# NinV/Background-Debiased-Video-CIL

Hardware: AMD Instinct MI355X
Metric: clips/sec fwd+bwd TSM-R50 8x224^2 bs32/GPU (higher is better)
Workload: dtype f32; 1 GPU; TSM-ResNet50 fwd+bwd+SGD step, synthetic 32x8x3x224x224 clips per GPU, 101 classes, SimpleLinear+CrossEntropyLoss, dropout 0.5, random-init weights; fp32 tensors, accumulators and results; conv products: fp32 via 3xbf16 split, 6 MFMA products, fp32 accumulate (dropped terms <= 2^-24 relative); conv_arith=bf16x3, clips_per_gpu=32, global_batch=32, parallelism=dp1

## Files before the change

background-debiased-video-cil_amd/_lib.py:

```python
from __future__ import annotations

import ctypes
import os
from ctypes import POINTER, Structure, c_char, c_char_p, c_float, c_int, c_int32, c_int64, c_size_t, c_uint16, c_uint64, c_void_p

_HERE = os.path.dirname(os.path.abspath(__file__))
_OVERRIDE = os.environ.get('BDVCIL_LIB_PATH')
LIB_PATH = _OVERRIDE or os.path.join(_HERE, 'csrc', 'libbdvcil_hip.so')
ABI_VERSION = 33

_lib = None


class ConvGeom(Structure):
    _fields_ = [(n, c_int32) for n in
                ('N', 'H', 'W', 'Cin', 'Ho', 'Wo', 'Cout', 'R', 'S', 'stride', 'pad', 'T', 'fold', 'pad_w', 'Rt', 'st_t', 'act_dtype')]

    def key(self):
        return tuple(getattr(self, n) for n, _ in self._fields_)


class ConvPlan(Structure):
    _fields_ = [(n, c_int32) for n in ('family', 'reads_planes', 'stat_rows', 'splits', 'pre_ok')] + [('kernel', c_char * 128)]

# ... 19 lines not shown
        return (self.width, self.height, self.ncomp, tuple(self.h), tuple(self.v))


SIGNATURES = {
    'bdv_last_error': (c_char_p, []),
    'bdv_abi_version': (c_int, []),
    'bdv_source_hash': (c_char_p, []),
    'bdv_conv_workspace_bytes': (c_size_t, [POINTER(ConvGeom), c_int]),
    'bdv_conv_plan_query': (c_int, [POINTER(ConvGeom), c_int, c_int, c_int, POINTER(ConvPlan)]),
    'bdv_conv_fprop': (c_int, [P, P, P, POINTER(ConvGeom), P, POINTER(ConvAffine), P, c_size_t, P]),
    'bdv_conv_dgrad': (c_int, [P, P, P, P, P, POINTER(ConvGeom), POINTER(BnStatFuse), P, c_size_t, P]),
    'bdv_conv_weight_planes_bytes': (c_size_t, [POINTER(ConvGeom)]),
    'bdv_conv_split_weights': (c_int, [P, POINTER(ConvGeom), P, P, P]),
    'bdv_conv_debug_force_tile': (c_int, [c_int]),
    'bdv_conv_debug_row_run': (c_int, [c_int]),
    'bdv_conv_fprop_pl': (c_int, [P, P, P, P, POINTER(ConvGeom), P, POINTER(ConvAffine), P, c_size_t, c_int, P, P, P]),
    'bdv_conv_dgrad_pl': (c_int, [P, P, P, P, P, P, POINTER(ConvGeom), POINTER(BnStatFuse), P, c_size_t, c_int, P]),
    'bdv_conv_wgrad': (c_int, [P, P, P, c_float, POINTER(ConvGeom), P, c_size_t, P]),
    'bdv_conv_wgrad_partial': (c_int, [P, P, POINTER(ConvGeom), P, c_size_t, P]),
    'bdv_conv_wgrad_partial_pl': (c_int, [P, P, POINTER(ConvGeom), P, c_size_t, c_int, P, P, P]),
    'bdv_wgrad_reduce_batched': (c_int, [P, P, P, P, c_int, c_float, P]),
    'bdv_f16x2_amax': (c_int, [P, c_int64, P, P]),
    'bdv_f16x2_scale': (c_float, [c_float]),
    'bdv_conv_split_weights_f16x2': (c_int, [P, POINTER(ConvGeom), P, P, P]),
    'bdv_conv_fprop_f16x2': (c_int, [P, P, P, P, P, POINTER(ConvGeom), P, POINTER(ConvAffine), P, c_size_t, P, P, P]),
    'bdv_conv_dgrad_f16x2': (c_int, [P, P, P, P, P, P, P, POINTER(ConvGeom), POINTER(BnStatFuse), P, c_size_t, P]),
    'bdv_conv_wgrad_partial_f16x2': (c_int, [P, P, P, P, POINTER(ConvGeom), P, c_size_t, P, P, P]),
    'bdv_bn_workspace_bytes': (c_size_t, [c_int64, c_int]),
    'bdv_bn_train_stats': (c_int, [P, c_int64, c_int, P, P, c_float, c_float, P, P, P, P, P, P, P, c_size_t, P]),
    'bdv_bn_train_finalize': (c_int, [P, c_int, c_int64, c_int, P, P, c_float, c_float, P, P, P, P, P, P, P]),
# ... 143 lines not shown
```

background-debiased-video-cil_amd/csrc/conv_mfma.hip:

```cpp
#include <stdlib.h>
#include <string.h>
#include "common.h"
#include "conv_row_run.h"

#ifdef BDV_STAMPS
__device__ unsigned long long* g_stamp_buf = nullptr;
__device__ int g_stamp_cap = 0;
#define BDV_STAMP(slot)                                                                                                          \
  do {                                                                                                                           \
    if (threadIdx.x == 0 && g_stamp_buf != nullptr && (int)(blockIdx.x + gridDim.x * blockIdx.y) < g_stamp_cap) {                 \
      unsigned long long* q_ = g_stamp_buf + (size_t)(blockIdx.x + gridDim.x * blockIdx.y) * 8;                                  \
      if ((slot) == 4) asm volatile("s_waitcnt vmcnt(0)" ::: "memory");                                                          \
      q_[slot] = __builtin_amdgcn_s_memtime();                                                                                   \
      if ((slot) == 0) { q_[5] = __builtin_amdgcn_s_memrealtime(); q_[7] = __builtin_amdgcn_s_getreg((4 << 0) | (0 << 6) | (31 << 11)); } \
      if ((slot) == 4) q_[6] = __builtin_amdgcn_s_memrealtime();                                                                 \
    }                                                                                                                            \
  } while (0)
#else
#define BDV_STAMP(slot) do { } while (0)
#endif

namespace {

constexpr int BK = 32;

struct Geom {
  int N, H, W, Cin, Ho, Wo, Cout, R, S, stride, pad, pad_w, T, fold;
  int Rt, st_t;
  float rcp_RS, rcp_S;
  int M;
  int Ktot;
  float rcp_HoWo, rcp_Wo;
  int stagger;
  int row_run;
};

typedef unsigned int u32x4 __attribute__((ext_vector_type(4)));
constexpr int kOOB = (int)0x80000000;

__device__ __forceinline__ float4 buf_load16(__amdgpu_buffer_rsrc_t rsrc, int voff, int soff) {
  const u32x4 v = __builtin_amdgcn_raw_buffer_load_b128(rsrc, voff, soff, 0);
  return make_float4(__uint_as_float(v.x), __uint_as_float(v.y), __uint_as_float(v.z), __uint_as_float(v.w));
}

__device__ __forceinline__ void buf_store16(__amdgpu_buffer_rsrc_t rsrc, int voff, float4 v) {
  u32x4 d;
  d.x = __float_as_uint(v.x);
  d.y = __float_as_uint(v.y);
  d.z = __float_as_uint(v.z);
  d.w = __float_as_uint(v.w);
  __builtin_amdgcn_raw_buffer_store_b128(d, rsrc, voff, 0, 0);
}
// ... 173 lines not shown
  const float* invstd;
  float* partial;
  int MT;
  const float* rscale;
  const float* rshift;
};

struct StatAcc {
  float4 s1, s2, mu, is;
  __device__ __forceinline__ void init(const BnStat& st, int col) {
    s1 = s2 = make_float4(0.f, 0.f, 0.f, 0.f);
    mu = *reinterpret_cast<const float4*>(st.mean + col);
    is = *reinterpret_cast<const float4*>(st.invstd + col);
  }
  __device__ __forceinline__ static unsigned sign_bits(const BnStat& st, int col, const float4 yv) {
    const float4 rsc = *reinterpret_cast<const float4*>(st.rscale + col), rsh = *reinterpret_cast<const float4*>(st.rshift + col);
    return (fmaf(yv.x, rsc.x, rsh.x) > 0.f ? 1u : 0u) | (fmaf(yv.y, rsc.y, rsh.y) > 0.f ? 2u : 0u) |
           (fmaf(yv.z, rsc.z, rsh.z) > 0.f ? 4u : 0u) | (fmaf(yv.w, rsc.w, rsh.w) > 0.f ? 8u : 0u);
  }
  __device__ __forceinline__ void accumulate(const float4 v, const float4 yv) {
    s1.x += v.x; s1.y += v.y; s1.z += v.z; s1.w += v.w;
    s2.x += v.x * ((yv.x - mu.x) * is.x);
    s2.y += v.y * ((yv.y - mu.y) * is.y);
    s2.z += v.z * ((yv.z - mu.z) * is.z);
    s2.w += v.w * ((yv.w - mu.w) * is.w);
  }
};

template <int BN, int NT = 256>
__device__ __forceinline__ void stat_flush(const StatAcc& a, const BnStat& st, float* __restrict__ smem, int Cin, int mt, int nt,
                                           int tid) {
// ... 31 lines not shown
    for (int j = 0; j < TN; ++j)
#pragma unroll
      for (int e = 0; e < 16; ++e) smem[(wm * 32 + acc_row(e, lane)) * BN + wn0 + 32 * WN * j + (lane & 31)] = acc[i][j][e];
    __syncthreads();
#pragma unroll
    for (int q = 0; q < PER; ++q) {
      const int idx = tid + NT * q;
      const int lr = idx / V, c4 = idx - lr * V;
      const float4 v = *reinterpret_cast<const float4*>(smem + lr * BN + 4 * c4);
      emit(32 * WM * i + lr, 4 * c4, v);
    }
  }
}


template <int BM, int BN, int WM, int WN, bool DERIVE = true, int ES = 4, bool PIPE = false, class RowMap>
__device__ __forceinline__ void dgrad_epilogue(const f32x16 (&acc)[BM / WM / 32][BN / WN / 32], float* __restrict__ smem, int tid,
                                               void* __restrict__ dx, const void* __restrict__ add_src,
                                               const uint32_t* __restrict__ add_mask, const Geom& g, int mt, int nt, int Mrows,
                                               const BnStat& stat, RowMap&& rowmap) {
  constexpr int TM = BM / WM / 32, TN = BN / WN / 32;
  constexpr int NT = 64 * WM * WN;
  constexpr int V = BN / 4;
  constexpr int PER = WM * 32 * V / NT;
  const int lane = tid & 63, wave = tid >> 6;
  const int wm = wave / WN, wn0 = (wave % WN) * 32;
  const int HW = g.H * g.W;
  const float rcp_HW = 1.0f / (float)HW;
  const int total_bytes = g.N * HW * g.Cin * ES;
  const int mask_bytes = g.N * HW * (g.Cin / 8);
  const __amdgpu_buffer_rsrc_t dxr = __builtin_amdgcn_make_buffer_rsrc((void*)dx, 0, total_bytes, 0x00020000);
  const __amdgpu_buffer_rsrc_t adr =
      __builtin_amdgcn_make_buffer_rsrc((void*)(add_src ? add_src : dx), 0, add_src ? total_bytes : 0, 0x00020000);
  const __amdgpu_buffer_rsrc_t amr =
      __builtin_amdgcn_make_buffer_rsrc((void*)(add_mask ? (const void*)add_mask : (const void*)dx), 0, add_mask ? mask_bytes : 0, 0x00020000);
  const bool do_stat = stat.y != nullptr;
  const __amdgpu_buffer_rsrc_t syr =
      __builtin_amdgcn_make_buffer_rsrc((void*)(do_stat ? stat.y : dx), 0, do_stat ? total_bytes : 0, 0x00020000);
  const __amdgpu_buffer_rsrc_t smr = __builtin_amdgcn_make_buffer_rsrc(
      (void*)(do_stat && stat.mask ? (const void*)stat.mask : (const void*)dx), 0, do_stat && stat.mask ? mask_bytes : 0, 0x00020000);
  const int col = nt * BN + 4 * (tid % V);
  const int cls = shift_class(col, g.fold);
  StatAcc sa;
  if (do_stat) sa.init(stat, col);
  constexpr int HB = PER < 4 ? PER : 4;
  constexpr int NBATCH = PER / HB;
  static_assert(PER % HB == 0, "pieces per pass must be whole batches");
  constexpr int NSETS = PIPE ? 2 : 1;
  float4 a[NSETS][HB], yv[NSETS][HB];
  uint32_t am[NSETS][HB], sm[NSETS][HB];
  int off[NSETS][HB];
  bool zero[NSETS][HB];
  auto issue = [&](int set, int i, int q0) __attribute__((always_inline)) {
#pragma unroll
    for (int u = 0; u < HB; ++u) {
      const int lr = (tid + NT * (q0 + u)) / V;
      const int mrow = mt * BM + 32 * WM * i + lr;
      const bool ok = mrow < Mrows;
      const int row = rowmap(ok ? mrow : 0);
      int drow = row;
      bool z = false;
      if (cls != 0) {
        int n, rem;
        fast_divmod(row, HW, rcp_HW, n, rem);
        const int t = n % g.T;
        const bool inside = (unsigned)(t + cls) < (unsigned)g.T;
        drow = inside ? row + cls * HW : row - cls * (g.T - 1) * HW;
        z = !inside;
      }
      const int o = drow * g.Cin + col;
      off[set][u] = ok ? o * ES : kOOB;
      zero[set][u] = z;
      a[set][u] = buf_ld4<ES>(adr, off[set][u]);
      am[set][u] = add_mask ? __builtin_amdgcn_raw_buffer_load_b32(amr, ok ? (o >> 5) << 2 : kOOB, 0, 0) : 0xffffffffu;
      if (do_stat) {
        yv[set][u] = buf_ld4<ES>(syr, off[set][u]);
        sm[set][u] = stat.mask ? __builtin_amdgcn_raw_buffer_load_b32(smr, ok ? (o >> 5) << 2 : kOOB, 0, 0) : 0xffffffffu;
      }
    }
  };
  auto finish = [&](int set, int q0) __attribute__((always_inline)) {
#pragma unroll
    for (int u = 0; u < HB; ++u) {
      const int lr = (tid + NT * (q0 + u)) / V;
      const float4 t4 = *reinterpret_cast<const float4*>(smem + lr * BN + 4 * (tid % V));
      const int sh = (off[set][u] / ES) & 31;
      const unsigned nib = (am[set][u] >> sh) & 0xFu;
      float4 r = zero[set][u] ? make_float4(0.f, 0.f, 0.f, 0.f) : t4;
      r.x += (nib & 1u) ? a[set][u].x : 0.f;
      r.y += (nib & 2u) ? a[set][u].y : 0.f;
      r.z += (nib & 4u) ? a[set][u].z : 0.f;
      r.w += (nib & 8u) ? a[set][u].w : 0.f;
      buf_st4<ES>(dxr, off[set][u], r);
      if (do_stat && off[set][u] != kOOB) {
        const unsigned sn = (DERIVE && stat.rscale != nullptr) ? StatAcc::sign_bits(stat, col, yv[set][u]) : (sm[set][u] >> sh) & 0xFu;
        float4 gq;
        gq.x = (sn & 1u) ? r.x : 0.f;
        gq.y = (sn & 2u) ? r.y : 0.f;
        gq.z = (sn & 4u) ? r.z : 0.f;
        gq.w = (sn & 8u) ? r.w : 0.f;
        sa.accumulate(gq, yv[set][u]);
      }
    }
  };
  if constexpr (PIPE) issue(0, 0, 0);
#pragma unroll
  for (int i = 0; i < TM; ++i) {
    __syncthreads();
#pragma unroll
    for (int j = 0; j < TN; ++j)
#pragma unroll
      for (int e = 0; e < 16; ++e) smem[(wm * 32 + acc_row(e, lane)) * BN + wn0 + 32 * WN * j + (lane & 31)] = acc[i][j][e];
    __syncthreads();
#pragma unroll
    for (int bq = 0; bq < NBATCH; ++bq) {
      if constexpr (PIPE) {
        const int b = i * NBATCH + bq;
        if (b + 1 < TM * NBATCH) issue((b + 1) & 1, (b + 1) / NBATCH, ((b + 1) % NBATCH) * HB);
        finish(b & 1, bq * HB);
      } else {
        issue(0, i, bq * HB);
        finish(0, bq * HB);
      }
    }
  }
  if (do_stat) stat_flush<BN, NT>(sa, stat, smem, g.Cin, blockIdx.y * (stat.MT >> (gridDim.y == 4 ? 2 : 0)) + mt, nt, tid);
}

// ... 528 lines not shown
struct DgradRowMap {
  int st, ph, pw, Wc, HcWc, H, W;
  __device__ __forceinline__ int operator()(int mrow) const {
    if (st == 1) return mrow;
    const int n = mrow / HcWc;
    const int rem = mrow - n * HcWc;
    const int hc = rem / Wc;
    return (n * H + hc * st + ph) * W + (rem - hc * Wc) * st + pw;
  }
};

template <class Stage, bool DERIVE, bool PIPE>
__device__ __forceinline__ void dgrad_tile(float* __restrict__ smem, const float* __restrict__ dy, const float* __restrict__ w,
                                           float* __restrict__ dx, const float* __restrict__ add_src,
                                           const uint32_t* __restrict__ add_mask, const Geom& g, int NT, const Work& wk,
                                           float* __restrict__ slab, const BnStat& stat) {
  constexpr int BM = Stage::BM, BN = Stage::BN, WM = Stage::WM, WN = Stage::WN;
  constexpr int TM = Stage::TM, TN = Stage::TN, AP = Stage::AP;

  const int st = g.stride;
  const int ph = blockIdx.y / st, pw = blockIdx.y - ph * st;
  const int Hc = (g.H - ph + st - 1) / st, Wc = (g.W - pw + st - 1) / st;
  const int Mc = g.N * Hc * Wc;
  const int MT = (Mc + BM - 1) / BM;
  const int r0 = (ph + g.pad) % st, s0 = (pw + g.pad_w) % st;
  const int nr = r0 < g.R ? (g.R - r0 + st - 1) / st : 0;
  const int ns = s0 < g.S ? (g.S - s0 + st - 1) / st : 0;
  const int bh = (ph + g.pad - r0) / st, bw = (pw + g.pad_w - s0) / st;
  const int ntap = nr * ns;
  const int nk = ntap * g.Cout / BK;

// ... 50 lines not shown
    const int tap = (r0 + k.ir * st) * g.S + (s0 + k.is * st);
    const int koff_a = (k.chunk * BK - (k.ir * g.Wo + k.is) * g.Cout) * 4;
    const int koff_b = Stage::kPlanes ? (tap * nchunk + k.chunk) * g.Cin * 64 : (k.chunk * BK * RS + tap) * g.Cin * 4;
#pragma unroll
    for (int p = 0; p < AP; ++p) {
      const bool v = (unsigned)(a_h[p] - k.ir) < (unsigned)g.Ho && (unsigned)(a_w[p] - k.is) < (unsigned)g.Wo;
      ra[p] = buf_load16(yr, (a_base[p] + koff_a) | (v ? 0 : kOOB), 0);
    }
    Stage::load_b(rb, wr, b_base, koff_b, plane_bytes);
    k.advance(ns, nr);
  };

  f32x16 acc[TM][TN];
  zero_acc<TM, TN>(acc);

  if (it.ke > it.kb) {
    load();
    for (int kt = it.kb; kt < it.ke; ++kt) {
      __syncthreads();
      Stage::store(smem, ra, rb, tid);
      __syncthreads();
      if (kt + 1 < it.ke) load();
      Stage::mma(smem, acc, wm0, wn0, lane);
    }
  }
  if (it.pslot >= 0) {
    store_partial<TM, TN>(slab, it.pslot, acc, tid);
    return;
  }

  dgrad_epilogue<BM, BN, WM, WN, DERIVE, 4, PIPE>(acc, smem, tid, dx, add_src, add_mask, g, mt, nt, Mc, stat, DgradRowMap{st, ph, pw, Wc, HcWc, g.H, g.W});
}

template <int BM, int BN, int WM, int WN>
__global__ __launch_bounds__(256, (F32Stage<BM, BN, WM, WN, false>::kOcc)) void conv_dgrad_kernel(const float* __restrict__ dy, const float* __restrict__ w,
                                                          float* __restrict__ dx, const float* __restrict__ add_src,
                                                          const uint32_t* __restrict__ add_mask, Geom g, int NT, Work wk,
                                                          float* __restrict__ slab, BnStat stat) {
  using Stage = F32Stage<BM, BN, WM, WN, false>;
  __shared__ __attribute__((aligned(16))) float smem[Stage::kSmemFloats];
  dgrad_tile<Stage, BN == 64, false>(smem, dy, w, dx, add_src, add_mask, g, NT, wk, slab, stat);
}

template <int BM, int BN, int WM, int WN, bool BPRE = false>
__global__ __launch_bounds__(256, (X3Stage<BM, BN, WM, WN, true>::kOcc)) void conv_dgrad_x3_kernel(const float* __restrict__ dy, const float* __restrict__ wt,
                                                          float* __restrict__ dx, const float* __restrict__ add_src,
                                                          const uint32_t* __restrict__ add_mask, Geom g, int NT, Work wk,
                                                          float* __restrict__ slab, BnStat stat) {
  static_assert(BPRE, "the weight operand of the bf16-piece kernels comes from the planes");
  using Stage = X3Stage<BM, BN, WM, WN, true>;
  __shared__ __attribute__((aligned(16))) float smem[Stage::kSmemFloats];
  dgrad_tile<Stage, true, true>(smem, dy, wt, dx, add_src, add_mask, g, NT, wk, slab, stat);
}

template <int BM, int BN, int WM, int WN>
__global__ __launch_bounds__(64 * WM * WN) void conv_dgrad_fixup_kernel(const float* __restrict__ slab, float* __restrict__ dx,
                                                                const float* __restrict__ add_src,
                                                                const uint32_t* __restrict__ add_mask, Geom g, int NT, Work wk,
                                                                BnStat stat) {
  constexpr int TM = BM / WM / 32, TN = BN / WN / 32;
  __shared__ __attribute__((aligned(16))) float smem[WM * 32 * BN];
  const int rt = blockIdx.x, tile = wk.dp_tiles + rt;
  const int mt = tile / NT, nt = tile - mt * NT;
  const int tid = threadIdx.x;
  f32x16 acc[TM][TN];
  load_partials<TM, TN, 64 * WM * WN>(slab, rt, wk.split, acc, tid);
  dgrad_epilogue<BM, BN, WM, WN>(acc, smem, tid, dx, add_src, add_mask, g, mt, nt, g.M, stat, [](int mrow) { return mrow; });
}

template <int BM, int BN, int WM, int WN, bool C4, bool INCR>
__global__ __launch_bounds__(256, 3) void conv_wgrad_kernel(const float* __restrict__ dy, const float* __restrict__ x,
                                                          float* __restrict__ slab, Geom g, int MTw, int NTw,
                                                          int kt_per_split) {
  constexpr int LDA = BM, LDB = BN;
  constexpr int TM = BM / WM / 32, TN = BN / WN / 32;
  constexpr int AP = BM / 32, BP = BN / 32;
  constexpr int AV = BM / 4, BV = BN / 4;
  __shared__ __attribute__((aligned(16))) float smem[BK * (LDA + LDB)];
  float* const As = smem;
  float* const Bs = smem + BK * LDA;

  const int tiles = MTw * NTw;
// ... 423 lines not shown
    tile[1][co_l][tx] = l16;
  }
  if (D == nullptr) return;
  __syncthreads();
#pragma unroll
  for (int p = 0; p < 4; ++p) {
    const int ci_l = ty + 8 * p;
    const size_t o = (((size_t)tap * (Cout >> 5) + (co0 >> 5)) * Cin + ci0 + ci_l) * 32 + tx;
    D[o] = tile[0][tx][ci_l];
    D[plane + o] = tile[1][tx][ci_l];
  }
}

using PlSet0 = std::integral_constant<int, 0>;
using PlSet1 = std::integral_constant<int, 1>;
template <typename LoadF, typename StoreF, typename MmaF>
__device__ __forceinline__ void pl_pipeline2(int n, LoadF&& load, StoreF&& store, MmaF&& mma, bool late = false) {
  load(PlSet0{});
  store(0, PlSet0{});
  if (n > 1) load(PlSet1{});
  if (n > 2) load(PlSet0{});
  __syncthreads();
  BDV_STAMP(1);
  int i = 0;
  if (late) {
    for (; i + 4 < n; i += 2) {
      store(1, PlSet1{});
      load(PlSet1{});
      mma(0);
      __syncthreads();
      store(0, PlSet0{});
      load(PlSet0{});
// ... 1 lines not shown
      __syncthreads();
    }
  } else {
    for (; i + 4 < n; i += 2) {
      mma(0);
      store(1, PlSet1{});
      load(PlSet1{});
      __syncthreads();
      mma(1);
      store(0, PlSet0{});
      load(PlSet0{});
      __syncthreads();
    }
  }
  for (; i < n; i += 2) {
    mma(0);
    if (i + 1 < n) store(1, PlSet1{});
    if (i + 3 < n) load(PlSet1{});
    __syncthreads();
    if (i + 1 >= n) break;
    mma(1);
    if (i + 2 < n) store(0, PlSet0{});
    if (i + 4 < n) load(PlSet0{});
    __syncthreads();
  }
}

constexpr int pl_waves_per_simd(int waves, int np, bool fits128) { return np == 1 && waves == 8 && fits128 ? 4 : waves == 4 ? 2 : waves / 4; }

constexpr int kRrRows = 256 + 96;
constexpr int kRrDataRows = kRrRows - 1;
template <int BM, int BN, int NP, int ES, bool PRE>
constexpr bool kRowRunTile = BM == 256 && BN == 64 && NP >= 2 && ES == 4 && !PRE;
template <int BM, int BN, int NP>
constexpr int kRowRunSmem = 2 * NP * (kRrRows * 64 + BN * 64);
// ... 373 lines not shown
                                                                                      void* __restrict__ dx,
                                                                                      const void* __restrict__ add_src,
                                                                                      const uint32_t* __restrict__ add_mask, Geom g,
                                                                                      int NT, Work wk, float* __restrict__ slab,
                                                                                      BnStat stat, PieceScales ps) {
  static_assert(!kF16<PT> || (NP == 2 && ES == 4), "fp16 pieces: two per operand, fp32 tensors");
  constexpr int NTHR = 64 * WM * WN;
  constexpr int TM = BM / WM / 32, TN = BN / WN / 32;
  constexpr int KG = ES == 2 ? 4 : 8;
  constexpr int AP = BM * KG / NTHR;
  constexpr int BPP = (BN * 4 + NTHR - 1) / NTHR;
  constexpr int PA = BM * 64, PB = BN * 64, STAGE = NP * (PA + PB);
  constexpr int SMEM0 = NBUF * STAGE >= WM * 32 * BN * 4 ? NBUF * STAGE : WM * 32 * BN * 4;
  constexpr bool RR = kRowRunTile<BM, BN, NP, ES, false> && NBUF == 2;
  constexpr int SMEM = RR && kRowRunSmem<BM, BN, NP> > SMEM0 ? kRowRunSmem<BM, BN, NP> : SMEM0;
  static_assert(AP >= 1 && SMEM <= 160 * 1024, "tile / epilogue staging do not fit");
  __shared__ __attribute__((aligned(16))) unsigned char smem_b[SMEM];
  float* const smem = reinterpret_cast<float*>(smem_b);

  BDV_STAMP(0);
  const int st = g.stride;
  const int ph = blockIdx.y / st, pw = blockIdx.y - ph * st;
  const int Hc = (g.H - ph + st - 1) / st, Wc = (g.W - pw + st - 1) / st;
  const int Mc = g.N * Hc * Wc;
  const int MT = (Mc + BM - 1) / BM;
  const int r0 = (ph + g.pad) % st, s0 = (pw + g.pad_w) % st;
  const int nr = r0 < g.R ? (g.R - r0 + st - 1) / st : 0;
  const int ns = s0 < g.S ? (g.S - s0 + st - 1) / st : 0;
  const int bh = (ph + g.pad - r0) / st, bw = (pw + g.pad_w - s0) / st;
  const int ntap = nr * ns;
  const int nk = ntap * g.Cout / BK;

// ... 155 lines not shown
        constexpr int SET = decltype(set)::value;
        if (b_active) {
#pragma unroll
          for (int pl = 0; pl < NP; ++pl)
#pragma unroll
            for (int q = 0; q < BPP; ++q)
              *reinterpret_cast<u32x4*>(Bst + stage * (NP * PB) + st_b + (pl * PB + (NTHR / 4) * q * 64)) = rb[SET][pl * BPP + q];
        }
      };
      pl_pipeline_rr(it.ke - it.kb, k.is, loadA, nextA, storeA, loadB, storeB, [&](int img, auto part, int stage) __attribute__((always_inline)) {
        mma_stage_rr<BM, BN, WM, WN, NP, PT, PAR>(smem_b + img * (NP * PAR), Bst + stage * (NP * PB), acc, fa3[2 - decltype(part)::value], fb);
      }, g.stagger != 0 && wave >= WM * WN / 2);
      rr_done = true;
    }
  }
  if (it.ke > it.kb && !rr_done) {
    if constexpr (NBUF == 2) {
      pl_pipeline2(it.ke - it.kb, load, store, [&](int stage) __attribute__((always_inline)) {
        mma_stage_pl<BM, BN, WM, WN, NP, PT>(smem_b + stage * STAGE, smem_b + stage * STAGE + NP * PA, acc, fa, fb);
      }, g.stagger != 0 && wave >= WM * WN / 2);
    } else {
      load(PlSet0{});
      for (int kt = it.kb; kt < it.ke; ++kt) {
        __syncthreads();
        store(0, PlSet0{});
        __syncthreads();
        if (kt == it.kb) BDV_STAMP(1);
        if (kt + 1 < it.ke) load(PlSet0{});
        mma_stage_pl<BM, BN, WM, WN, NP, PT>(smem_b, smem_b + NP * PA, acc, fa, fb);
      }
    }
  }
  BDV_STAMP(2);
  f16x2_unscale<PT>(acc, ps);
  if (it.pslot >= 0) {
    store_partial<TM, TN, NTHR>(slab, it.pslot, acc, tid);
    return;
  }
  constexpr bool EPI_PIPE = TM * TN <= 4 && NP >= 2 && BM != 64;
  dgrad_epilogue<BM, BN, WM, WN, true, ES, EPI_PIPE>(acc, smem, tid, dx, add_src, add_mask, g, mt, nt, Mc, stat, DgradRowMap{st, ph, pw, Wc, HcWc, g.H, g.W});
  BDV_STAMP(3);
  BDV_STAMP(4);
}

typedef short s16x4_t __attribute__((ext_vector_type(4)));

template <int COLS, int NP = 3, int ROWS = 32, typename PT = Bf16Pieces>
__device__ __forceinline__ void pl_store_rows(unsigned char* __restrict__ base, int krow, int c4, const float4 v, float scale = 1.f) {
  constexpr int PITCH = 2 * COLS + 64, PLANE = ROWS * PITCH;
  if constexpr (kF16<PT>) {
    static_assert(NP == 2, "fp16 pieces: two per operand");
    u32x2_t hi, lo;
    split2_f16_pairs(v, scale, hi, lo);
    unsigned char* q = base + krow * PITCH + 8 * c4;
    *reinterpret_cast<u32x2_t*>(q) = hi;
// ... 276 lines not shown
  }
  if (g->fold > 0) {
    BDV_REQUIRE(g->fold % 4 == 0 && 2 * g->fold <= g->Cin, "%s: fold=%d must be a multiple of 4 and <= Cin/2", who,
                g->fold);
    BDV_REQUIRE(g->T > 0 && g->N % g->T == 0, "%s: N=%d not a multiple of T=%d", who, g->N, g->T);
    BDV_REQUIRE(g->Cin % BK == 0, "%s: temporal shift needs Cin %% 32 == 0", who);
  }
  BDV_REQUIRE((int64_t)g->N * g->H * g->W * g->Cin < (1ll << 29) && (int64_t)g->N * g->Ho * g->Wo * g->Cout < (1ll << 29),
              "%s: tensor exceeds 2^29 elements", who);
  BDV_REQUIRE((int64_t)g->Cout * g->R * g->S * g->Cin < (1ll << 29), "%s: weight tensor too large", who);
  BDV_REQUIRE((int64_t)g->N * g->Ho * g->Wo < (1ll << 22) || g->Cin == 4, "%s: more than 2^22 output pixels", who);
  return BDV_OK;
}

int g_pl_row_run = 1;
static bool pl_stagger_enabled() {
  const char* e = getenv("BDVCIL_STAGGER");
  return e == nullptr || atoi(e) != 0;
}

Geom make_geom(const bdv_conv_geom* g) {
  Geom d;
  d.stagger = pl_stagger_enabled() ? 1 : 0;
  d.row_run = g_pl_row_run;
  d.N = g->N; d.H = g->H; d.W = g->W; d.Cin = g->Cin; d.Ho = g->Ho; d.Wo = g->Wo; d.Cout = g->Cout;
  d.R = g->R; d.S = g->S; d.stride = g->stride; d.pad = g->pad; d.pad_w = g->pad_w < 0 ? g->pad : g->pad_w;
  d.T = (g->fold > 0 || g->Rt > 1) ? g->T : 1;
  d.fold = g->fold;
  d.Rt = g->Rt > 1 ? g->Rt : 1;
  d.st_t = g->Rt > 1 ? g->st_t : 1;
  d.rcp_RS = 1.0f / (float)(g->R * g->S);
  d.rcp_S = 1.0f / (float)g->S;
  d.M = 0; d.Ktot = 0;
  d.rcp_HoWo = 1.0f / (float)(g->Ho * g->Wo);
  d.rcp_Wo = 1.0f / (float)g->Wo;
  return d;
}

bool debug_plan() {
// ... 549 lines not shown
    char tiles[256] = "";
    for (int t = 0, n = 0; t < kNumPlTiles && n < (int)sizeof(tiles); ++t) {
      const PlTile& k = kPlTiles[t];
      n += snprintf(tiles + n, sizeof(tiles) - n, "%d = %dx%d%s, ", t, k.BM, k.BN, !k.fprop ? " (dgrad)" : k.WM * k.WN == 4 ? " (four waves)" : "");
    }
    bdv_set_error("bdv_conv_debug_force_tile: cfg %d (-1 automatic, %s%d = none)", cfg, tiles, kNumPlTiles);
    return BDV_EINVAL;
  }
  g_pl_tile_forced = cfg;
  return BDV_OK;
}

extern "C" int bdv_conv_debug_row_run(int on) {
  BDV_REQUIRE(on == 0 || on == 1, "bdv_conv_debug_row_run: on = %d (1 = one activation image per filter row, 0 = the per-tap loader)", on);
  g_pl_row_run = on;
  return BDV_OK;
}

extern "C" int bdv_conv_split_weights(const float* w, const bdv_conv_geom* gg, void* planes_fprop, void* planes_dgrad, void* stream) {
  if (int e = check_geom(gg, "bdv_conv_split_weights")) return e;
  BDV_REQUIRE(w && (planes_fprop || planes_dgrad), "bdv_conv_split_weights: null pointer");
  BDV_REQUIRE(gg->Cin % 32 == 0 && gg->Cout % 32 == 0, "bdv_conv_split_weights: Cin=%d and Cout=%d must be multiples of 32", gg->Cin, gg->Cout);
  BDV_REQUIRE(bdv_aligned16(w) && bdv_aligned16(planes_fprop) && bdv_aligned16(planes_dgrad), "bdv_conv_split_weights: alignment");
  const dim3 grid(gg->Cin / 32, gg->Cout / 32, gg->R * gg->S);
  hipLaunchKernelGGL(split_weights_kernel, grid, dim3(256), 0, (hipStream_t)stream, w, (unsigned short*)planes_fprop,
                     (unsigned short*)planes_dgrad, gg->Cout, gg->R * gg->S, gg->Cin);
  BDV_LAUNCH_CHECK("bdv_conv_split_weights");
  return BDV_OK;
}

// ... 460 lines not shown
```

background-debiased-video-cil_amd/kernels.py:

```python
from __future__ import annotations

import ctypes
from typing import Optional, Sequence, Tuple

import torch

from ._lib import BnStatFuse, ConvAffine, ConvGeom, ConvPlan, check, lib

_WS = {}


def _stream():
    return ctypes.c_void_p(torch.cuda.current_stream().cuda_stream)


def _p(t: Optional[torch.Tensor]):
    return ctypes.c_void_p(0 if t is None else t.data_ptr())


def _chk(t: torch.Tensor, shape: Optional[Sequence[int]] = None, dtype=torch.float32, name='tensor'):
    if not isinstance(t, torch.Tensor):
        raise TypeError(f'{name}: expected a tensor, got {type(t)}')
    if not t.is_cuda:
        raise RuntimeError(f'{name}: the HIP path needs a GPU tensor (got device {t.device}); there is no CPU fallback')
# ... 427 lines not shown
        planes_d = weight_planes(w, g, f16)[1] if plan.reads_planes else None
        check(lib().bdv_conv_dgrad_f16x2(_p(dy), _p(act_amax(dy) if f16 else None), _p(w), _p(planes_d), _p(dx), _p(add_src),
                                         _p(add_mask_src), ctypes.byref(g), ctypes.byref(fuse) if fuse is not None else None, _p(ws),
                                         ws.numel(), _stream()), 'bdv_conv_dgrad_f16x2')
    elif use_x3:
        planes_d = weight_planes(w, g)[1] if plan.reads_planes else None
        check(lib().bdv_conv_dgrad_pl(_p(dy), _p(w), _p(planes_d), _p(dx), _p(add_src), _p(add_mask_src), ctypes.byref(g),
                                      ctypes.byref(fuse) if fuse is not None else None, _p(ws), ws.numel(), PIECES, _stream()),
              'bdv_conv_dgrad_pl')
    else:
        check(lib().bdv_conv_dgrad(_p(dy), _p(w), _p(dx), _p(add_src), _p(add_mask_src), ctypes.byref(g),
                                   ctypes.byref(fuse) if fuse is not None else None, _p(ws), ws.numel(), _stream()), 'bdv_conv_dgrad')
    return dx if bn_stats is None else (dx, partial)


def conv_wgrad(dy: torch.Tensor, x: torch.Tensor, g: ConvGeom, dw: Optional[torch.Tensor] = None,
               beta: float = 0.0, ws_tag: str = 'wgrad', x3: Optional[bool] = None, pre_bn=None) -> torch.Tensor:
    g.act_dtype = _act_code(dy)
    _chk_conv(dy, (g.N, g.Ho, g.Wo, g.Cout), g, 'dy')
    _chk_conv(x, (_in_frames(g), g.H, g.W, g.Cin), g, 'x')
    if dw is None:
        dw = torch.empty((g.Cout, _taps_r(g), g.S, g.Cin), dtype=torch.float32, device=dy.device)
        beta = 0.0
    _chk(dw, (g.Cout, _taps_r(g), g.S, g.Cin), name='dw')
    if WGRAD_X3 if x3 is None else x3:
        slab, _ = conv_wgrad_partial(dy, x, g, x3=True, dw=dw, pre_bn=pre_bn)
        wgrad_reduce_batched([(slab, dw)], beta=beta)
        return dw
    _chk_bf16_arith(g, False, 'conv_wgrad')
    conv_plan(g, 'wgrad', False, pre_bn is not None)
# ... 1225 lines not shown
```

include/bdvcil_hip.h:

```cpp
#ifndef BDVCIL_HIP_H
#define BDVCIL_HIP_H

#include <stddef.h>
#include <stdint.h>

#ifdef __cplusplus
extern "C" {
#endif

#define BDV_OK 0
#define BDV_EINVAL (-1)
#define BDV_EWORKSPACE (-2)

#define BDV_ACT_F32 0
#define BDV_ACT_BF16 1

typedef struct bdv_conv_geom {
  int32_t N;
  int32_t H, W;
  int32_t Cin;
  int32_t Ho, Wo;
  int32_t Cout;
  int32_t R, S;
  int32_t stride;
// ... 44 lines not shown
  const float* mean;
  const float* invstd;
  float* partial;
  const float* relu_scale;
  const float* relu_shift;
} bdv_bn_stat_fuse;

int bdv_conv_dgrad(const float* dy, const float* w, float* dx, const float* add_src,
                   const uint32_t* add_mask_src, const bdv_conv_geom* g, const bdv_bn_stat_fuse* bn_stat, void* workspace,
                   size_t workspace_bytes, void* stream);

size_t bdv_conv_weight_planes_bytes(const bdv_conv_geom* g);
int bdv_conv_split_weights(const float* w, const bdv_conv_geom* g, void* planes_fprop, void* planes_dgrad, void* stream);
int bdv_conv_debug_force_tile(int cfg);
int bdv_conv_debug_row_run(int on);
int bdv_conv_fprop_pl(const void* x, const float* w, const void* planes_fprop, void* y, const bdv_conv_geom* g,
                      float* bn_partial, const bdv_conv_affine* affine, void* workspace, size_t workspace_bytes, int pieces,
                      const float* pre_scale, const float* pre_shift, void* stream);
int bdv_conv_dgrad_pl(const void* dy, const float* w, const void* planes_dgrad, void* dx, const void* add_src,
                      const uint32_t* add_mask_src, const bdv_conv_geom* g, const bdv_bn_stat_fuse* bn_stat, void* workspace,
                      size_t workspace_bytes, int pieces, void* stream);

#define BDV_ARITH_F16X2 4
int bdv_f16x2_amax(const float* t, int64_t n, void* amax, void* stream);
float bdv_f16x2_scale(float amax);
int bdv_conv_split_weights_f16x2(const float* w, const bdv_conv_geom* g, void* planes_fprop, void* planes_dgrad, void* stream);
int bdv_conv_fprop_f16x2(const void* x, const void* amax_x, const float* w, const void* planes_fprop, void* y,
                         const bdv_conv_geom* g, float* bn_partial, const bdv_conv_affine* affine, void* workspace,
                         size_t workspace_bytes, const float* pre_scale, const float* pre_shift, void* stream);
int bdv_conv_dgrad_f16x2(const void* dy, const void* amax_dy, const float* w, const void* planes_dgrad, void* dx,
// ... 228 lines not shown
```

Before: 624.0 clips/s.

## Warm dgrad epilogue operand lines from the last K step via buffer-to-LDS loads

During the final K iteration of the dgrad kernels, each thread issues buffer_load_lds prefetches of the epilogue's first-pass operands (add source, add mask, BN stat y and mask) into a scratch LDS area. The goal is to bring those cache lines in while the last MMA runs, so the epilogue's global reads hit cache. The epilogue also stages the ReLU rescale/shift vectors in LDS instead of re-reading them from global per piece, and replaces its __syncthreads with an lgkmcnt-only barrier. The cost is extra LDS per block, which can lower occupancy, plus extra memory traffic. A debug toggle can turn the warming off.

```diff
diff --git a/background-debiased-video-cil_amd/_lib.py b/background-debiased-video-cil_amd/_lib.py
--- a/background-debiased-video-cil_amd/_lib.py
+++ b/background-debiased-video-cil_amd/_lib.py
@@ -57,6 +57,7 @@
     'bdv_conv_split_weights': (c_int, [P, POINTER(ConvGeom), P, P, P]),
     'bdv_conv_debug_force_tile': (c_int, [c_int]),
     'bdv_conv_debug_row_run': (c_int, [c_int]),
+    'bdv_conv_debug_epilogue_warm': (c_int, [c_int]),
     'bdv_conv_fprop_pl': (c_int, [P, P, P, P, POINTER(ConvGeom), P, POINTER(ConvAffine), P, c_size_t, c_int, P, P, P]),
     'bdv_conv_dgrad_pl': (c_int, [P, P, P, P, P, P, POINTER(ConvGeom), POINTER(BnStatFuse), P, c_size_t, c_int, P]),
     'bdv_conv_wgrad': (c_int, [P, P, P, c_float, POINTER(ConvGeom), P, c_size_t, P]),
diff --git a/background-debiased-video-cil_amd/csrc/conv_mfma.hip b/background-debiased-video-cil_amd/csrc/conv_mfma.hip
--- a/background-debiased-video-cil_amd/csrc/conv_mfma.hip
+++ b/background-debiased-video-cil_amd/csrc/conv_mfma.hip
@@ -33,9 +33,11 @@
   float rcp_HoWo, rcp_Wo;
   int stagger;
   int row_run;
+  int epi_warm;
 };
 
 typedef unsigned int u32x4 __attribute__((ext_vector_type(4)));
+typedef __attribute__((address_space(3))) void* lds_ptr_t;
 constexpr int kOOB = (int)0x80000000;
 
 __device__ __forceinline__ float4 buf_load16(__amdgpu_buffer_rsrc_t rsrc, int voff, int soff) {
@@ -239,7 +241,9 @@
     is = *reinterpret_cast<const float4*>(st.invstd + col);
   }
   __device__ __forceinline__ static unsigned sign_bits(const BnStat& st, int col, const float4 yv) {
-    const float4 rsc = *reinterpret_cast<const float4*>(st.rscale + col), rsh = *reinterpret_cast<const float4*>(st.rshift + col);
+    return sign_bits(*reinterpret_cast<const float4*>(st.rscale + col), *reinterpret_cast<const float4*>(st.rshift + col), yv);
+  }
+  __device__ __forceinline__ static unsigned sign_bits(const float4 rsc, const float4 rsh, const float4 yv) {
     return (fmaf(yv.x, rsc.x, rsh.x) > 0.f ? 1u : 0u) | (fmaf(yv.y, rsc.y, rsh.y) > 0.f ? 2u : 0u) |
            (fmaf(yv.z, rsc.z, rsh.z) > 0.f ? 4u : 0u) | (fmaf(yv.w, rsc.w, rsh.w) > 0.f ? 8u : 0u);
   }
@@ -301,11 +305,74 @@
 }
 
 
+__device__ __forceinline__ __amdgpu_buffer_rsrc_t dgrad_operand_rsrc(const void* p, void* dx, int bytes) {
+  return __builtin_amdgcn_make_buffer_rsrc(p ? (void*)p : dx, 0, p ? bytes : 0, 0x00020000);
+}
+
+template <int BM, int WM, class RowMap>
+__device__ __forceinline__ int dgrad_piece_row(const Geom& g, int mt, int i, int lr, int cls, int Mrows, int HW, float rcp_HW,
+                                               const RowMap& rowmap, bool& ok, bool& z) {
+  const int mrow = mt * BM + 32 * WM * i + lr;
+  ok = mrow < Mrows;
+  const int row = rowmap(ok ? mrow : 0);
+  int drow = row;
+  z = false;
+  if (cls != 0) {
+    int n, rem;
+    fast_divmod(row, HW, rcp_HW, n, rem);
+    const int t = n % g.T;
+    const bool inside = (unsigned)(t + cls) < (unsigned)g.T;
+    drow = inside ? row + cls * HW : row - cls * (g.T - 1) * HW;
+    z = !inside;
+  }
+  return drow;
+}
+
+template <int BM, int BN, int WM, int WN, int ES, class RowMap>
+__device__ __forceinline__ void dgrad_warm_pass(unsigned* __restrict__ warm, int tid, void* __restrict__ dx,
+                                                const void* __restrict__ add_src, const uint32_t* __restrict__ add_mask, const Geom& g,
+                                                int mt, int nt, int Mrows, const BnStat& stat, const RowMap& rowmap, int i) {
+  static_assert((BN * ES) % 128 == 0, "a tile row is whole 128-byte lines");
+  constexpr int NT = 64 * WM * WN;
+  constexpr int L = BN * ES / 128;
+  constexpr int LINES = WM * 32 * L;
+  constexpr int CNT = (LINES + NT - 1) / NT;
+  const int HW = g.H * g.W;
+  const float rcp_HW = 1.0f / (float)HW;
+  const int total_bytes = g.N * HW * g.Cin * ES;
+  const int mask_bytes = g.N * HW * (g.Cin / 8);
+  const bool do_stat = stat.y != nullptr;
+  const __amdgpu_buffer_rsrc_t adr = dgrad_operand_rsrc(add_src, dx, total_bytes);
+  const __amdgpu_buffer_rsrc_t amr = dgrad_operand_rsrc(add_mask, dx, mask_bytes);
+  const __amdgpu_buffer_rsrc_t syr = dgrad_operand_rsrc(stat.y, dx, total_bytes);
+  const __amdgpu_buffer_rsrc_t smr = dgrad_operand_rsrc(do_stat ? stat.mask : nullptr, dx, mask_bytes);
+  const lds_ptr_t dst = (lds_ptr_t)(warm + 64 * (tid >> 6));
+#pragma unroll
+  for (int q = 0; q < CNT; ++q) {
+    const int idx = tid + NT * q;
+    const int lr = idx / L;
+    const int col = nt * BN + (idx - lr * L) * (128 / ES);
+    bool ok, z;
+    const int drow = dgrad_piece_row<BM, WM>(g, mt, i, lr, shift_class(col, g.fold), Mrows, HW, rcp_HW, rowmap, ok, z);
+    if (LINES % NT != 0) ok = ok && idx < LINES;
+    const int o = drow * g.Cin + col;
+    const int off = ok ? o * ES : kOOB, moff = ok ? (o >> 5) << 2 : kOOB;
+    if (add_src) __builtin_amdgcn_raw_ptr_buffer_load_lds(adr, dst, 4, off, 0, 0, 0);
+    if (add_mask) __builtin_amdgcn_raw_ptr_buffer_load_lds(amr, dst, 4, moff, 0, 0, 0);
+    if (do_stat) __builtin_amdgcn_raw_ptr_buffer_load_lds(syr, dst, 4, off, 0, 0, 0);
+    if (do_stat && stat.mask) __builtin_amdgcn_raw_ptr_buffer_load_lds(smr, dst, 4, moff, 0, 0, 0);
+  }
+}
+
+__device__ __forceinline__ void lds_only_barrier() { asm volatile("s_waitcnt lgkmcnt(0)\n\ts_barrier" ::: "memory"); }
+
+constexpr int dgrad_epi_words(int nthr, int bn) { return nthr + 2 * bn; }
+
 template <int BM, int BN, int WM, int WN, bool DERIVE = true, int ES = 4, bool PIPE = false, class RowMap>
 __device__ __forceinline__ void dgrad_epilogue(const f32x16 (&acc)[BM / WM / 32][BN / WN / 32], float* __restrict__ smem, int tid,
                                                void* __restrict__ dx, const void* __restrict__ add_src,
                                                const uint32_t* __restrict__ add_mask, const Geom& g, int mt, int nt, int Mrows,
-                                               const BnStat& stat, RowMap&& rowmap) {
+                                               const BnStat& stat, RowMap&& rowmap, unsigned* __restrict__ epi) {
   constexpr int TM = BM / WM / 32, TN = BN / WN / 32;
   constexpr int NT = 64 * WM * WN;
   constexpr int V = BN / 4;
@@ -317,19 +384,21 @@
   const int total_bytes = g.N * HW * g.Cin * ES;
   const int mask_bytes = g.N * HW * (g.Cin / 8);
   const __amdgpu_buffer_rsrc_t dxr = __builtin_amdgcn_make_buffer_rsrc((void*)dx, 0, total_bytes, 0x00020000);
-  const __amdgpu_buffer_rsrc_t adr =
-      __builtin_amdgcn_make_buffer_rsrc((void*)(add_src ? add_src : dx), 0, add_src ? total_bytes : 0, 0x00020000);
-  const __amdgpu_buffer_rsrc_t amr =
-      __builtin_amdgcn_make_buffer_rsrc((void*)(add_mask ? (const void*)add_mask : (const void*)dx), 0, add_mask ? mask_bytes : 0, 0x00020000);
+  const __amdgpu_buffer_rsrc_t adr = dgrad_operand_rsrc(add_src, dx, total_bytes);
+  const __amdgpu_buffer_rsrc_t amr = dgrad_operand_rsrc(add_mask, dx, mask_bytes);
   const bool do_stat = stat.y != nullptr;
-  const __amdgpu_buffer_rsrc_t syr =
-      __builtin_amdgcn_make_buffer_rsrc((void*)(do_stat ? stat.y : dx), 0, do_stat ? total_bytes : 0, 0x00020000);
-  const __amdgpu_buffer_rsrc_t smr = __builtin_amdgcn_make_buffer_rsrc(
-      (void*)(do_stat && stat.mask ? (const void*)stat.mask : (const void*)dx), 0, do_stat && stat.mask ? mask_bytes : 0, 0x00020000);
+  const __amdgpu_buffer_rsrc_t syr = dgrad_operand_rsrc(stat.y, dx, total_bytes);
+  const __amdgpu_buffer_rsrc_t smr = dgrad_operand_rsrc(do_stat ? stat.mask : nullptr, dx, mask_bytes);
   const int col = nt * BN + 4 * (tid % V);
   const int cls = shift_class(col, g.fold);
   StatAcc sa;
   if (do_stat) sa.init(stat, col);
+  const bool derive = DERIVE && do_stat && stat.rscale != nullptr;
+  float* const aff = epi != nullptr ? reinterpret_cast<float*>(epi + NT) : nullptr;
+  if (derive && aff != nullptr && tid < V) {
+    *reinterpret_cast<float4*>(aff + 4 * tid) = *reinterpret_cast<const float4*>(stat.rscale + col);
+    *reinterpret_cast<float4*>(aff + BN + 4 * tid) = *reinterpret_cast<const float4*>(stat.rshift + col);
+  }
   constexpr int HB = PER < 4 ? PER : 4;
   constexpr int NBATCH = PER / HB;
   static_assert(PER % HB == 0, "pieces per pass must be whole batches");
@@ -342,19 +411,8 @@
 #pragma unroll
     for (int u = 0; u < HB; ++u) {
       const int lr = (tid + NT * (q0 + u)) / V;
-      const int mrow = mt * BM + 32 * WM * i + lr;
-      const bool ok = mrow < Mrows;
-      const int row = rowmap(ok ? mrow : 0);
-      int drow = row;
-      bool z = false;
-      if (cls != 0) {
-        int n, rem;
-        fast_divmod(row, HW, rcp_HW, n, rem);
-        const int t = n % g.T;
-        const bool inside = (unsigned)(t + cls) < (unsigned)g.T;
-        drow = inside ? row + cls * HW : row - cls * (g.T - 1) * HW;
-        z = !inside;
-      }
+      bool ok, z;
+      const int drow = dgrad_piece_row<BM, WM>(g, mt, i, lr, cls, Mrows, HW, rcp_HW, rowmap, ok, z);
       const int o = drow * g.Cin + col;
       off[set][u] = ok ? o * ES : kOOB;
       zero[set][u] = z;
@@ -380,7 +438,12 @@
       r.w += (nib & 8u) ? a[set][u].w : 0.f;
       buf_st4<ES>(dxr, off[set][u], r);
       if (do_stat && off[set][u] != kOOB) {
-        const unsigned sn = (DERIVE && stat.rscale != nullptr) ? StatAcc::sign_bits(stat, col, yv[set][u]) : (sm[set][u] >> sh) & 0xFu;
+        unsigned sn = (sm[set][u] >> sh) & 0xFu;
+        if (derive) {
+          sn = aff != nullptr ? StatAcc::sign_bits(*reinterpret_cast<const float4*>(aff + 4 * (tid % V)),
+                                                   *reinterpret_cast<const float4*>(aff + BN + 4 * (tid % V)), yv[set][u])
+                              : StatAcc::sign_bits(stat, col, yv[set][u]);
+        }
         float4 gq;
         gq.x = (sn & 1u) ? r.x : 0.f;
         gq.y = (sn & 2u) ? r.y : 0.f;
@@ -393,12 +456,12 @@
   if constexpr (PIPE) issue(0, 0, 0);
 #pragma unroll
   for (int i = 0; i < TM; ++i) {
-    __syncthreads();
+    lds_only_barrier();
 #pragma unroll
     for (int j = 0; j < TN; ++j)
 #pragma unroll
       for (int e = 0; e < 16; ++e) smem[(wm * 32 + acc_row(e, lane)) * BN + wn0 + 32 * WN * j + (lane & 31)] = acc[i][j][e];
-    __syncthreads();
+    lds_only_barrier();
 #pragma unroll
     for (int bq = 0; bq < NBATCH; ++bq) {
       if constexpr (PIPE) {
@@ -957,7 +1020,7 @@
 __device__ __forceinline__ void dgrad_tile(float* __restrict__ smem, const float* __restrict__ dy, const float* __restrict__ w,
                                            float* __restrict__ dx, const float* __restrict__ add_src,
                                            const uint32_t* __restrict__ add_mask, const Geom& g, int NT, const Work& wk,
-                                           float* __restrict__ slab, const BnStat& stat) {
+                                           float* __restrict__ slab, const BnStat& stat, unsigned* __restrict__ warm) {
   constexpr int BM = Stage::BM, BN = Stage::BN, WM = Stage::WM, WN = Stage::WN;
   constexpr int TM = Stage::TM, TN = Stage::TN, AP = Stage::AP;
 
@@ -1038,6 +1101,8 @@
   f32x16 acc[TM][TN];
   zero_acc<TM, TN>(acc);
 
+  const DgradRowMap rowmap{st, ph, pw, Wc, HcWc, g.H, g.W};
+  const bool warm_on = g.epi_warm != 0 && it.pslot < 0;
   if (it.ke > it.kb) {
     load();
     for (int kt = it.kb; kt < it.ke; ++kt) {
@@ -1045,6 +1110,7 @@
       Stage::store(smem, ra, rb, tid);
       __syncthreads();
       if (kt + 1 < it.ke) load();
+      else if (warm_on) dgrad_warm_pass<BM, BN, WM, WN, 4>(warm, tid, dx, add_src, add_mask, g, mt, nt, Mc, stat, rowmap, 0);
       Stage::mma(smem, acc, wm0, wn0, lane);
     }
   }
@@ -1053,7 +1119,7 @@
     return;
   }
 
-  dgrad_epilogue<BM, BN, WM, WN, DERIVE, 4, PIPE>(acc, smem, tid, dx, add_src, add_mask, g, mt, nt, Mc, stat, DgradRowMap{st, ph, pw, Wc, HcWc, g.H, g.W});
+  dgrad_epilogue<BM, BN, WM, WN, DERIVE, 4, PIPE>(acc, smem, tid, dx, add_src, add_mask, g, mt, nt, Mc, stat, rowmap, warm);
 }
 
 template <int BM, int BN, int WM, int WN>
@@ -1063,7 +1129,8 @@
                                                           float* __restrict__ slab, BnStat stat) {
   using Stage = F32Stage<BM, BN, WM, WN, false>;
   __shared__ __attribute__((aligned(16))) float smem[Stage::kSmemFloats];
-  dgrad_tile<Stage, BN == 64, false>(smem, dy, w, dx, add_src, add_mask, g, NT, wk, slab, stat);
+  __shared__ __attribute__((aligned(16))) unsigned warm[dgrad_epi_words(256, BN)];
+  dgrad_tile<Stage, BN == 64, false>(smem, dy, w, dx, add_src, add_mask, g, NT, wk, slab, stat, warm);
 }
 
 template <int BM, int BN, int WM, int WN, bool BPRE = false>
@@ -1074,7 +1141,8 @@
   static_assert(BPRE, "the weight operand of the bf16-piece kernels comes from the planes");
   using Stage = X3Stage<BM, BN, WM, WN, true>;
   __shared__ __attribute__((aligned(16))) float smem[Stage::kSmemFloats];
-  dgrad_tile<Stage, true, true>(smem, dy, wt, dx, add_src, add_mask, g, NT, wk, slab, stat);
+  __shared__ __attribute__((aligned(16))) unsigned warm[dgrad_epi_words(256, BN)];
+  dgrad_tile<Stage, true, true>(smem, dy, wt, dx, add_src, add_mask, g, NT, wk, slab, stat, warm);
 }
 
 template <int BM, int BN, int WM, int WN>
@@ -1087,9 +1155,14 @@
   const int rt = blockIdx.x, tile = wk.dp_tiles + rt;
   const int mt = tile / NT, nt = tile - mt * NT;
   const int tid = threadIdx.x;
+  constexpr bool EPI_LDS = BM != 64;
+  __shared__ __attribute__((aligned(16))) unsigned epi_words[EPI_LDS ? dgrad_epi_words(64 * WM * WN, BN) : 4];
+  unsigned* const warm = EPI_LDS ? epi_words : nullptr;
+  const auto rowmap = [](int mrow) { return mrow; };
+  if (EPI_LDS && g.epi_warm != 0) dgrad_warm_pass<BM, BN, WM, WN, 4>(warm, tid, dx, add_src, add_mask, g, mt, nt, g.M, stat, rowmap, 0);
   f32x16 acc[TM][TN];
   load_partials<TM, TN, 64 * WM * WN>(slab, rt, wk.split, acc, tid);
-  dgrad_epilogue<BM, BN, WM, WN>(acc, smem, tid, dx, add_src, add_mask, g, mt, nt, g.M, stat, [](int mrow) { return mrow; });
+  dgrad_epilogue<BM, BN, WM, WN>(acc, smem, tid, dx, add_src, add_mask, g, mt, nt, g.M, stat, rowmap, warm);
 }
 
 template <int BM, int BN, int WM, int WN, bool C4, bool INCR>
@@ -1543,8 +1616,11 @@
 
 using PlSet0 = std::integral_constant<int, 0>;
 using PlSet1 = std::integral_constant<int, 1>;
-template <typename LoadF, typename StoreF, typename MmaF>
-__device__ __forceinline__ void pl_pipeline2(int n, LoadF&& load, StoreF&& store, MmaF&& mma, bool late = false) {
+struct PlNoLastStep {
+  __device__ __forceinline__ void operator()() const {}
+};
+template <typename LoadF, typename StoreF, typename MmaF, typename LastF = PlNoLastStep>
+__device__ __forceinline__ void pl_pipeline2(int n, LoadF&& load, StoreF&& store, MmaF&& mma, bool late = false, LastF&& last_step = LastF{}) {
   load(PlSet0{});
   store(0, PlSet0{});
   if (n > 1) load(PlSet1{});
@@ -1576,11 +1652,13 @@
     }
   }
   for (; i < n; i += 2) {
+    if (i + 1 >= n) last_step();
     mma(0);
     if (i + 1 < n) store(1, PlSet1{});
     if (i + 3 < n) load(PlSet1{});
     __syncthreads();
     if (i + 1 >= n) break;
+    if (i + 2 >= n) last_step();
     mma(1);
     if (i + 2 < n) store(0, PlSet0{});
     if (i + 4 < n) load(PlSet0{});
@@ -1984,8 +2062,9 @@
   constexpr int SMEM0 = NBUF * STAGE >= WM * 32 * BN * 4 ? NBUF * STAGE : WM * 32 * BN * 4;
   constexpr bool RR = kRowRunTile<BM, BN, NP, ES, false> && NBUF == 2;
   constexpr int SMEM = RR && kRowRunSmem<BM, BN, NP> > SMEM0 ? kRowRunSmem<BM, BN, NP> : SMEM0;
-  static_assert(AP >= 1 && SMEM <= 160 * 1024, "tile / epilogue staging do not fit");
+  static_assert(AP >= 1 && SMEM + dgrad_epi_words(NTHR, BN) * 4 <= 160 * 1024, "tile / epilogue staging and the epilogue's words do not fit");
   __shared__ __attribute__((aligned(16))) unsigned char smem_b[SMEM];
+  __shared__ __attribute__((aligned(16))) unsigned warm[dgrad_epi_words(NTHR, BN)];
   float* const smem = reinterpret_cast<float*>(smem_b);
 
   BDV_STAMP(0);
@@ -2171,11 +2250,18 @@
       rr_done = true;
     }
   }
+  constexpr bool EPI_LDS = !(NP == 1 && ES == 4 && BM == 256 && BN == 64);
+  constexpr bool WARM_K = !(NP == 3 && BM * BN >= 128 * 256 && BN >= 128) && EPI_LDS;
+  const DgradRowMap rowmap{st, ph, pw, Wc, HcWc, g.H, g.W};
+  const bool warm_on = WARM_K && g.epi_warm != 0 && it.pslot < 0;
+  auto warm0 = [&]() __attribute__((always_inline)) {
+    if (warm_on) dgrad_warm_pass<BM, BN, WM, WN, ES>(warm, tid, dx, add_src, add_mask, g, mt, nt, Mc, stat, rowmap, 0);
+  };
   if (it.ke > it.kb && !rr_done) {
     if constexpr (NBUF == 2) {
       pl_pipeline2(it.ke - it.kb, load, store, [&](int stage) __attribute__((always_inline)) {
         mma_stage_pl<BM, BN, WM, WN, NP, PT>(smem_b + stage * STAGE, smem_b + stage * STAGE + NP * PA, acc, fa, fb);
-      }, g.stagger != 0 && wave >= WM * WN / 2);
+      }, g.stagger != 0 && wave >= WM * WN / 2, warm0);
     } else {
       load(PlSet0{});
       for (int kt = it.kb; kt < it.ke; ++kt) {
@@ -2184,6 +2270,7 @@
         __syncthreads();
         if (kt == it.kb) BDV_STAMP(1);
         if (kt + 1 < it.ke) load(PlSet0{});
+        else warm0();
         mma_stage_pl<BM, BN, WM, WN, NP, PT>(smem_b, smem_b + NP * PA, acc, fa, fb);
       }
     }
@@ -2195,7 +2282,7 @@
     return;
   }
   constexpr bool EPI_PIPE = TM * TN <= 4 && NP >= 2 && BM != 64;
-  dgrad_epilogue<BM, BN, WM, WN, true, ES, EPI_PIPE>(acc, smem, tid, dx, add_src, add_mask, g, mt, nt, Mc, stat, DgradRowMap{st, ph, pw, Wc, HcWc, g.H, g.W});
+  dgrad_epilogue<BM, BN, WM, WN, true, ES, EPI_PIPE>(acc, smem, tid, dx, add_src, add_mask, g, mt, nt, Mc, stat, rowmap, EPI_LDS ? warm : nullptr);
   BDV_STAMP(3);
   BDV_STAMP(4);
 }
@@ -2502,6 +2589,7 @@
 }
 
 int g_pl_row_run = 1;
+int g_epi_warm = 1;
 static bool pl_stagger_enabled() {
   const char* e = getenv("BDVCIL_STAGGER");
   return e == nullptr || atoi(e) != 0;
@@ -2511,6 +2599,7 @@
   Geom d;
   d.stagger = pl_stagger_enabled() ? 1 : 0;
   d.row_run = g_pl_row_run;
+  d.epi_warm = g_epi_warm;
   d.N = g->N; d.H = g->H; d.W = g->W; d.Cin = g->Cin; d.Ho = g->Ho; d.Wo = g->Wo; d.Cout = g->Cout;
   d.R = g->R; d.S = g->S; d.stride = g->stride; d.pad = g->pad; d.pad_w = g->pad_w < 0 ? g->pad : g->pad_w;
   d.T = (g->fold > 0 || g->Rt > 1) ? g->T : 1;
@@ -3090,6 +3179,12 @@
 extern "C" int bdv_conv_debug_row_run(int on) {
   BDV_REQUIRE(on == 0 || on == 1, "bdv_conv_debug_row_run: on = %d (1 = one activation image per filter row, 0 = the per-tap loader)", on);
   g_pl_row_run = on;
+  return BDV_OK;
+}
+
+extern "C" int bdv_conv_debug_epilogue_warm(int on) {
+  BDV_REQUIRE(on == 0 || on == 1, "bdv_conv_debug_epilogue_warm: on = %d (1 = the dgrad epilogues' first pass is warmed from the K loop, 0 = not)", on);
+  g_epi_warm = on;
   return BDV_OK;
 }
 
diff --git a/background-debiased-video-cil_amd/kernels.py b/background-debiased-video-cil_amd/kernels.py
--- a/background-debiased-video-cil_amd/kernels.py
+++ b/background-debiased-video-cil_amd/kernels.py
@@ -465,6 +465,10 @@
     return dx if bn_stats is None else (dx, partial)
 
 
+def conv_debug_epilogue_warm(on: bool) -> None:
+    check(lib().bdv_conv_debug_epilogue_warm(int(bool(on))), 'bdv_conv_debug_epilogue_warm')
+
+
 def conv_wgrad(dy: torch.Tensor, x: torch.Tensor, g: ConvGeom, dw: Optional[torch.Tensor] = None,
                beta: float = 0.0, ws_tag: str = 'wgrad', x3: Optional[bool] = None, pre_bn=None) -> torch.Tensor:
     g.act_dtype = _act_code(dy)
diff --git a/include/bdvcil_hip.h b/include/bdvcil_hip.h
--- a/include/bdvcil_hip.h
+++ b/include/bdvcil_hip.h
@@ -82,6 +82,7 @@
 int bdv_conv_split_weights(const float* w, const bdv_conv_geom* g, void* planes_fprop, void* planes_dgrad, void* stream);
 int bdv_conv_debug_force_tile(int cfg);
 int bdv_conv_debug_row_run(int on);
+int bdv_conv_debug_epilogue_warm(int on);
 int bdv_conv_fprop_pl(const void* x, const float* w, const void* planes_fprop, void* y, const bdv_conv_geom* g,
                       float* bn_partial, const bdv_conv_affine* affine, void* workspace, size_t workspace_bytes, int pieces,
                       const float* pre_scale, const float* pre_shift, void* stream);
```

Result: no change. 623.6 clips/s (-0.1%).
